# isl-org/Open3D-PointNet2-Semantic3D

Measured on AMD Instinct MI355X. Metric: points/sec through SA+FP stack (B=16,N=8192), higher is better.
Workload: dtype f32

## Files before the change

include/pn2_abi.h:

```cpp
#ifndef PN2_ABI_H_
#define PN2_ABI_H_

#include <stddef.h>
#include <stdint.h>

#ifdef __cplusplus
extern "C" {
#endif

#define PN2_ABI_VERSION 2

#define PN2_OK 0
#define PN2_EINVAL (-1)
#define PN2_ENULL (-2)
#define PN2_ERANGE (-3)
#define PN2_EUNSUP (-4)

#define PN2_ARITH_STRICT 0
#define PN2_ARITH_FMA 1
#define PN2_ARITH_FMA_ALT 2

int pn2_abi_version(void);
const char *pn2_build_info(void);
const char *pn2_strerror(int code);
// ... 157 lines not shown

size_t pn2_interpolate_label_workspace_bytes(int num_sparse_points);
int pn2_interpolate_label_with_color(int num_sparse_points, int num_dense_points,
                                     const float *sparse_points, const int *sparse_labels,
                                     const float *dense_points, int *dense_labels,
                                     uint8_t *dense_colors, int knn, void *workspace,
                                     size_t workspace_bytes, void *stream);


int pn2_linear_dgrad(int rows, int cin, int cout, const float *dy, const float *w, float *dx, void *stream);
int pn2_linear_dgrad_bn_grad_stats(int rows, int cin, int cout, const float *dy, const float *w, float *dx,
                                   const float *y_below, const float *gamma, const float *beta, const float *save_mean,
                                   const float *save_invstd, int relu, void *bn_workspace, size_t workspace_bytes,
                                   void *stream);

int pn2_weighted_ce_forward(int rows, int num_class, const float *logits, const void *labels, int label64,
                            const float *weights, float *lse, double *acc, float *loss, void *stream);
int pn2_weighted_ce_backward(int rows, int num_class, const float *logits, const void *labels, int label64,
                             const float *weights, const float *lse, const double *acc, const float *gout,
                             float *dlogits, void *stream);

int pn2_confusion_update(int rows, int num_class, const float *logits, const void *labels, int label64, int *pred,
                         long long *confusion, long long *invalid, const float *loss, double *loss_acc, void *stream);

int pn2_label_confusion(long long n, int num_class, const void *gt, const void *pd, int label64,
                        long long *confusion, long long *dropped, void *stream);

int pn2_dropout(long long n, const float *x, float keep_prob, const long long *state, float *y,
                unsigned char *mask, void *stream);
int pn2_dropout_grad(long long n, const float *dy, const unsigned char *mask, float keep_prob, float *dx,
                     void *stream);

int pn2_relu_grad(long long n, const float *z, const float *dz, float *dx, void *stream);

int pn2_adam_step(long long n, float *params, const float *grads, float *m, float *v, const float *hyper,
                  void *stream);

int pn2_momentum_step(long long n, float *params, const float *grads, float *accum, const float *hyper, void *stream);

int pn2_sa_group_concat(int b, int n, int m, int nsample, int c, const float *xyz, const float *new_xyz,
                        const float *points, const int *idx, float *out, void *stream);


int pn2_scene_extract_z_box(int n, const double *points, int b, const double *centers, double half_x,
                            double half_y, double scene_z_size, int cap, int *out_idx, int *out_cnt,
                            void *stream);

int pn2_scene_sample(int b, int npts, int cap, const double *points, const int *labels, const double *colors,
                     const int *idx, const int *cnt, const unsigned char *mask, double half_x, double half_y,
                     int *out_sel, float *out_centered, double *out_raw, int *out_labels, float *out_colors,
                     int *status, void *stream);

size_t pn2_voxel_downsample_workspace_bytes(int n);
int pn2_voxel_downsample(int n, const double *points, const double *colors, const int *labels, double voxel_size,
                         double *out_points, double *out_colors, int *out_labels, int *out_count, int *status,
                         void *workspace, size_t workspace_bytes, void *stream);

int pn2_dataset_workspace_size(int b, int max_chunks, unsigned long long *bytes);
int pn2_dataset_sample(int b, int npts, int num_scenes, int max_chunks, int use_color, int augment, const double *points,
                       const float *colors, const unsigned char *labels, const int *scene_offsets, const double *scene_cdf,
                       const double *scene_z_size, const float *label_weights, int num_label_weights, double half_x,
                       double half_y, unsigned long long seed, long long *counter, const int *draw_scene,
                       const int *draw_center, const unsigned char *draw_mask, int mask_cap, const double *draw_rot,
                       void *workspace, size_t workspace_bytes, int *out_info, double *out_finfo, int *out_sel,
                       float *out_data, int *out_labels, float *out_weights, void *stream);

int pn2_scene_ingest_workspace_size(int n, unsigned long long *bytes);
int pn2_scene_ingest(int n, const double *points, const double *colors, const int *labels, double *out_points,
                     float *out_colors, unsigned char *out_labels, int *out_perm, double *out_zrange, long long *out_hist,
                     int *status, void *workspace, size_t workspace_bytes, void *stream);

int pn2_fp_mlp_fused_pre(int b, int n, int m, int c1, const float *dist, const int *idx, const float *points1,
                         const float *z, int nlayers, const int *widths, const float *const *w,
                         const float *const *bias, float *y, void *stream);
int pn2_fp_mlp_fused_pre_ld(int b, int n, int m, int c1, const float *dist, const int *idx, const float *points1,
                            int ld_points1, const float *z, int nlayers, const int *widths, const float *const *w,
                            const float *const *bias, float *y, void *stream);

int pn2_fp_mlp_fused_pre_schedule(int b, int n, int m, int c1, const float *dist, const int *idx, const float *points1,
                                  const float *z, int nlayers, const int *widths, const float *const *w,
                                  const float *const *bias, float *y, int schedule, void *stream);

int pn2_set_sa_row_packing(int on);

int pn2_sa_mlp_fused_pre(int b, int n, int m, int nsample, const float *xyz, const float *new_xyz, const float *zf,
                         const int *idx, int nlayers, const int *widths, const float *const *w,
                         const float *const *bias, int pool, float *out, void *stream);

int pn2_fp_mlp_wide_pre(int b, int n, int m, int c1, const float *dist, const int *idx, const float *points1,
                        const float *z, int nlayers, const int *widths, const float *const *w,
                        const float *const *bias, float *y, void *stream);
int pn2_sa_mlp_wide_pre(int b, int n, int m, int nsample, const float *xyz, const float *new_xyz, const float *zf,
                        const int *idx, int nlayers, const int *widths, const float *const *w,
                        const float *const *bias, int pool, float *y, void *stream);

size_t pn2_ball_query_bin_bytes(int n);
int pn2_ball_query_bin(int b, int n, float radius, const float *xyz1, void *workspace, size_t workspace_bytes, void *stream);
int pn2_ball_query_bin_ld(int b, int n, float radius, const float *xyz1, int ld1, void *workspace, size_t workspace_bytes,
                          void *stream);
int pn2_query_ball_point_binned(int b, int n, int m, float radius, int nsample, const float *xyz1, const float *xyz2,
                                const void *bins, int *idx, int *pts_cnt, int arith_mode, void *stream);

int pn2_group_pool(long long rows, int k, int c, int mode, const float *x, const float *gxyz, float *out, void *stream);
int pn2_group_pool_grad(long long rows, int k, int c, int mode, const float *x, const float *gxyz, const float *dout,
                        float *dx, void *stream);

int pn2_bn_relu_forward_deferred(long long rows, int c, const float *y, const float *gamma, const float *beta,
                                 const float *bias, float eps, float decay, int stats_done, float *running_mean,
                                 float *running_var, void *workspace, size_t workspace_bytes, float *save_mean,
                                 float *save_invstd, float *scale, float *shift, void *stream);
int pn2_linear_bn_stats_xf(int rows, int cin, int cout, const float *x_raw, const float *w, float *y, void *bn_workspace,
                           size_t workspace_bytes, const float *a_scale, const float *a_shift, int a_relu, void *stream);
int pn2_linear_wgrad_accumulate_xf(int rows, int cin, int cout, const float *x_raw, const float *dy, float *dw,
                                   const float *a_scale, const float *a_shift, int a_relu, void *stream);

int pn2_linear_narrow(int rows, int cin, int cout, const float *x, const float *w, const float *bias, float *y, void *stream);

int pn2_bn_grad_constants(long long rows, int c, const float *dz, const float *y, const float *gamma, const float *beta,
                          const float *save_mean, const float *save_invstd, int relu, int pool, const float *zmax,
                          const float *ties, const float *ysel, int stats_done, void *workspace, size_t workspace_bytes,
                          float *coef, float *dgamma, float *dbeta, void *stream);
int pn2_bn_relu_forward_pool(long long rows, int c, const float *y, const float *gamma, const float *beta, const float *bias,
                             float eps, float decay, int relu, int pool, float *running_mean, float *running_var,
                             void *workspace, size_t workspace_bytes, int stats_mode, float *save_mean, float *save_invstd,
                             float *zmax, float *ties, float *ysel, void *stream);
int pn2_linear_dgrad_gx(int rows, int cin, int cout, const float *y, const float *dz, const float *coef, int relu, int pool,
                        const float *zmax, const float *ties, const float *w, float *dx, const float *y_below,
                        const float *gamma_below, const float *beta_below, const float *mean_below, const float *invstd_below,
                        int relu_below, void *ws_below, size_t ws_below_bytes, void *stream);
int pn2_linear_wgrad_gx(int rows, int cin, int cout, const float *x, const float *a_scale, const float *a_shift, int a_relu,
                        const float *y, const float *dz, const float *coef, int relu, int pool, const float *zmax,
                        const float *ties, float *dw, void *stream);

int pn2_linear_bn_stats_fin(int rows, int cin, int cout, const float *x, const float *w, float *y, void *bn_workspace,
                            size_t workspace_bytes, const float *a_scale, const float *a_shift, int a_relu, int finish,
                            const float *gamma, const float *beta, const float *bias, float eps, float decay,
                            float *running_mean, float *running_var, float *save_mean, float *save_invstd, float *scale,
                            float *shift, void *stream);
int pn2_linear_dgrad_fin(int rows, int cin, int cout, const float *dy, const float *y, const float *dz, const float *coef,
                         int relu, int pool, const float *zmax, const float *ties, const float *w, float *dx,
                         const float *y_below, const float *gamma_below, const float *beta_below, const float *mean_below,
                         const float *invstd_below, int relu_below, void *ws_below, size_t ws_below_bytes, int finish_below,
                         float *coef_below, float *dgamma_below, float *dbeta_below, void *stream);
int pn2_bn_relu_forward_mode(long long rows, int c, const float *y, const float *gamma, const float *beta, const float *bias,
                             float eps, float decay, int relu, float *running_mean, float *running_var, void *workspace,
                             size_t workspace_bytes, int stats_mode, float *save_mean, float *save_invstd, float *z,
                             void *stream);
int pn2_bn_relu_backward_mode(long long rows, int c, const float *dz, const float *y, const float *gamma, const float *beta,
                              const float *save_mean, const float *save_invstd, int relu, int pool, const float *zmax,
                              const float *ties, void *workspace, size_t workspace_bytes, int stats_mode, float *dy,
                              float *dgamma, float *dbeta, void *stream);

int pn2_linear_bwd_fused(int rows, int cin, int cout, const float *x, const float *a_scale, const float *a_shift, int a_relu,
                         const float *y, const float *dz, const float *coef, int relu, int pool, const float *zmax,
                         const float *ties, const float *w, float *dx, float *dw, const float *y_below,
                         const float *gamma_below, const float *beta_below, const float *mean_below, const float *invstd_below,
                         int relu_below, void *ws_below, size_t ws_below_bytes, int finish_below, float *coef_below,
                         float *dgamma_below, float *dbeta_below, void *stream);

int pn2_sa_first_layer_bn(int b, int n, int m, int nsample, int c, int cout, const float *xyz, const float *new_xyz,
                          const float *points, const int *idx, const float *w, float *y, float *xg, void *workspace,
                          size_t workspace_bytes, int finish, const float *gamma, const float *beta, const float *bias, float eps,
                          float decay, float *running_mean, float *running_var, float *save_mean, float *save_invstd,
                          float *scale, float *shift, void *stream);

int pn2_sa_hoist_rows(int b, int n, int m, int nsample, int cout, const float *xyz, const float *new_xyz, const int *idx,
// ... 134 lines not shown
```

open3d-pointnet2-semantic3d_amd/csrc/pn2_mlp_wide.hip:

```cpp
#include "pn2_common.h"
#include "pn2_layer_stack.h"

namespace {

typedef float f32x4 __attribute__((ext_vector_type(4)));
typedef float f32x16 __attribute__((ext_vector_type(16)));

constexpr int kWideDepth = 4;

struct WideParams {
    int rows, cin, x_stride, nlayers, pool, relu_last;
    int w[3];
    const float* x;
    int n, m, c;
    const float* xyz;
    const float* new_xyz;
    const float* points;
    const int* idx;
    const float* dist;
    const float* points1;
    int c1, c2;
    const float* W[3];
    const float* bias[3];
    float* y;
    const float* zpre;
    int rowtab_off;
    int sa[2];
    int scratch_off;
    int scratch_alias;
};

enum { kWidePlain = 0, kWideGather = 1, kWideInterp = 2 };
constexpr int kPackChunk = 256;
constexpr int kPackRows = 0, kPackGroups = 32, kPackMeta = 36, kPackCounts = 40, kPackLdsInts = 64;
template <int MODE, bool PACK = false>
__global__ void __launch_bounds__(256, 2)
mlp_wide_kernel(WideParams p) {
    constexpr bool GATHER = MODE == kWideGather;
    static_assert(!PACK || GATHER, "PACK: the pooled gather mode only");
    extern __shared__ __attribute__((aligned(16))) float smem[];
    const int tid = threadIdx.x;
    const int lane = tid & 63, half = lane >> 5, l31 = lane & 31;
    const int wave = __builtin_amdgcn_readfirstlane(tid >> 6);
    const int tile = blockIdx.x;
    const int row0 = tile * 32;
    const int buf_off[2] = {0, 32 * p.sa[0]};
    float* const buf0 = smem;

    struct LayerCfg { int N, wnt, ks_n, nq, ks, cb, g0, g1; const float* wcol; };
    auto make_cfg = [&](int l, int Kt) {
        LayerCfg c;
        c.N = p.w[l];
        c.wnt = c.N >> 7;
        c.ks_n = 4 / c.wnt;
        c.nq = wave % c.wnt;
        c.ks = wave / c.wnt;
        c.cb = c.nq * 128;
        const int ngroups = (Kt + 7) >> 3;
        c.g0 = (ngroups * c.ks) / c.ks_n;
        c.g1 = (ngroups * (c.ks + 1)) / c.ks_n;
        c.wcol = p.W[l] + c.cb + 4 * l31;
        return c;
    };
    f32x4 bq[kWideDepth][4];
    auto fetch_b = [&](const LayerCfg& c, int g, f32x4 (&b_)[4]) {
        const float* __restrict__ wp = c.wcol + (size_t)(8 * g + 4 * half) * c.N;
#pragma unroll
        for (int q = 0; q < 4; ++q) b_[q] = *reinterpret_cast<const f32x4*>(wp + (size_t)q * c.N);
    };
    auto prefetch_b = [&](const LayerCfg& c) {
#pragma unroll
        for (int u = 0; u < kWideDepth; ++u) fetch_b(c, c.g0 + u < c.g1 ? c.g0 + u : c.g1 - 1, bq[u]);
    };
    const LayerCfg first = make_cfg(0, p.cin);
    int* const pk = reinterpret_cast<int*>(smem + p.rowtab_off);
    (void)pk;
    if constexpr (PACK) {
        const int groups = p.rows >> 5;
        const int cbase = (tile / kPackChunk) * kPackChunk, mytile = tile - cbase;
        const int cnt = min(kPackChunk, groups - cbase);
        int cls = 0;
        if (tid < cnt) {
            const int4* __restrict__ ip = reinterpret_cast<const int4*>(p.idx + (size_t)(cbase + tid) * 32);
            int4 v[8];
#pragma unroll
            for (int u = 0; u < 8; ++u) v[u] = ip[u];
            const int head = v[0].x;
            int live = 1;
#pragma unroll
            for (int u = 0; u < 8; ++u) {
                if (v[u].x != head) live = 4 * u + 1;
                if (v[u].y != head) live = 4 * u + 2;
                if (v[u].z != head) live = 4 * u + 3;
                if (v[u].w != head) live = 4 * u + 4;
            }
            cls = live <= 8 ? 8 : (live <= 16 ? 16 : 32);
        }
        const unsigned long long m32 = __ballot(cls == 32), m16 = __ballot(cls == 16), m8 = __ballot(cls == 8);
        if (lane == 0) {
            pk[kPackCounts + 3 * wave + 0] = __popcll(m32);
            pk[kPackCounts + 3 * wave + 1] = __popcll(m16);
            pk[kPackCounts + 3 * wave + 2] = __popcll(m8);
        }
        __syncthreads();
        int n32 = 0, n16 = 0, n8 = 0, b32 = 0, b16 = 0, b8 = 0;
#pragma unroll
        for (int w = 0; w < 4; ++w) {
            const int c32 = pk[kPackCounts + 3 * w], c16 = pk[kPackCounts + 3 * w + 1], c8 = pk[kPackCounts + 3 * w + 2];
            n32 += c32; n16 += c16; n8 += c8;
            if (w < wave) { b32 += c32; b16 += c16; b8 += c8; }
        }
        n32 = __builtin_amdgcn_readfirstlane(n32); n16 = __builtin_amdgcn_readfirstlane(n16); n8 = __builtin_amdgcn_readfirstlane(n8);
        const int promote = ((n16 & 1) && (n8 & 3) == 1) ? 1 : 0;
        const int k16 = n16 + promote, k8 = n8 - promote, t16 = (k16 + 1) >> 1;
        const int ntiles = n32 + t16 + ((k8 + 3) >> 2);
        if (mytile >= ntiles) return;
        prefetch_b(first);
        if (cls != 0) {
            const unsigned long long below = (1ull << lane) - 1ull;
            int t, slot;
            if (cls == 32) { t = b32 + __popcll(m32 & below); slot = 0; }
            else {
                int c = cls, r = cls == 16 ? b16 + __popcll(m16 & below) : b8 + __popcll(m8 & below);
                if (promote && c == 8 && r == n8 - 1) { c = 16; r = n16; }
                if (c == 16) { t = n32 + (r >> 1); slot = r & 1; }
                else { t = n32 + t16 + (r >> 2); slot = r & 3; }
            }
            if (t == mytile) pk[kPackGroups + slot] = cbase + tid;
        }
        if (tid == 0) {
            int sshift, nvalid;
            if (mytile < n32) { sshift = 5; nvalid = 1; }
            else if (mytile < n32 + t16) { sshift = 4; nvalid = min(2, k16 - 2 * (mytile - n32)); }
            else { sshift = 3; nvalid = min(4, k8 - 4 * (mytile - n32 - t16)); }
            pk[kPackMeta] = sshift; pk[kPackMeta + 1] = nvalid;
        }
        __syncthreads();
    } else {
        prefetch_b(first);
    }

    const int K0 = (p.cin + 7) & ~7;
    auto stage4 = [&](int count4, int cv, int sa, auto src_of) {
        for (int base = 0; base < count4; base += 256 * 8) {
            f32x4 v[8];
#pragma unroll
            for (int u = 0; u < 8; ++u) {
                int e = base + u * 256 + tid;
                e = e < count4 ? e : count4 - 1;
                const int r = e / cv, j = e - r * cv;
                v[u] = *reinterpret_cast<const f32x4*>(src_of(r, j));
            }
#pragma unroll
            for (int u = 0; u < 8; ++u) {
                const int e = base + u * 256 + tid;
// ... 75 lines not shown
            for (int u = 0; u < 4; ++u) {
                const int e = base + u * 256 + tid;
                if (e < count4) {
                    const int r = e / cv2, j = e - r * cv2;
                    *reinterpret_cast<f32x4*>(buf0 + r * p.sa[0] + 4 * j) = v[u];
                }
            }
        }
        if (c1 > 0) {
            const float* __restrict__ p1 = p.points1 + (size_t)row0 * c1;
            for (int e = tid; e < 32 * cv1; e += 256) {
                const int r = e / cv1, j = e - r * cv1;
                *reinterpret_cast<f32x4*>(buf0 + r * p.sa[0] + (p.zpre ? 0 : c2) + 4 * j) = *reinterpret_cast<const f32x4*>(p1 + (size_t)r * c1 + 4 * j);
            }
        }
        if (K0 > p.cin) {
            const int padw = K0 - p.cin;
            for (int e = tid; e < 32 * padw; e += 256) buf0[(e / padw) * p.sa[0] + p.cin + e % padw] = 0.f;
        }
    } else {
        const float* __restrict__ x = p.x;
        if ((p.x_stride & 3) == 0 && (p.cin & 3) == 0 && (((uintptr_t)x) & 15) == 0) {
            const int cv = p.cin >> 2;
            stage4(32 * cv, cv, p.sa[0], [&](int r, int j) {
                const int gr = row0 + r < p.rows ? row0 + r : p.rows - 1;
                return x + (size_t)gr * p.x_stride + 4 * j;
            });
            if (row0 + 32 > p.rows) {
                __syncthreads();
                for (int e = tid; e < 32 * p.cin; e += 256) {
                    const int r = e / p.cin;
                    if (row0 + r >= p.rows) buf0[r * p.sa[0] + e - r * p.cin] = 0.f;
                }
            }
        } else {
            const int total = 32 * p.cin;
            for (int base = 0; base < total; base += 256 * 8) {
                float v[8];
#pragma unroll
                for (int u = 0; u < 8; ++u) {
                    int e = base + u * 256 + tid;
                    e = e < total ? e : total - 1;
                    const int r = e / p.cin, k = e - r * p.cin;
                    const int gr = row0 + r < p.rows ? row0 + r : p.rows - 1;
                    v[u] = x[(size_t)gr * p.x_stride + k];
                }
#pragma unroll
                for (int u = 0; u < 8; ++u) {
                    const int e = base + u * 256 + tid;
                    if (e < total) {
                        const int r = e / p.cin, k = e - r * p.cin;
                        buf0[r * p.sa[0] + k] = row0 + r < p.rows ? v[u] : 0.f;
                    }
                }
            }
        }
        if (K0 > p.cin) {
            const int padw = K0 - p.cin;
            for (int e = tid; e < 32 * padw; e += 256) buf0[(e / padw) * p.sa[0] + p.cin + e % padw] = 0.f;
        }
    }
    __syncthreads();

    LayerCfg cur = first;
#pragma unroll 1
    for (int l = 0; l < p.nlayers; ++l) {
        const int N = cur.N, wnt = cur.wnt, ks_n = cur.ks_n, nq = cur.nq, ks = cur.ks, cb = cur.cb, g0 = cur.g0, g1 = cur.g1;
        const int in_off = buf_off[l & 1];
        const int sin = p.sa[l & 1];
        const float* __restrict__ arow = smem + in_off + l31 * sin + 4 * half;

        f32x16 acc[4];
#pragma unroll
        for (int t = 0; t < 4; ++t)
#pragma unroll
            for (int r = 0; r < 16; ++r) acc[t][r] = 0.f;

        auto contract = [&](const f32x4& a_, const f32x4 (&b_)[4]) {
#pragma unroll
            for (int q = 0; q < 4; ++q)
#pragma unroll
                for (int t = 0; t < 4; ++t) acc[t] = __builtin_amdgcn_mfma_f32_32x32x2f32(a_[q], b_[q][t], acc[t], 0, 0, 0);
        };
        if (g0 < g1) {
            const int last = g1 - 1;
            f32x4 aq[kWideDepth];
#pragma unroll
            for (int u = 0; u < kWideDepth; ++u) aq[u] = *reinterpret_cast<const f32x4*>(arow + 8 * (g0 + u < g1 ? g0 + u : last));
            int g = g0;
            for (; g + 2 * kWideDepth <= g1; g += kWideDepth) {
#pragma unroll
                for (int u = 0; u < kWideDepth; ++u) {
                    contract(aq[u], bq[u]);
                    __builtin_amdgcn_sched_barrier(0);
                    const int gn = g + kWideDepth + u;
                    aq[u] = *reinterpret_cast<const f32x4*>(arow + 8 * gn);
                    fetch_b(cur, gn, bq[u]);
                    __builtin_amdgcn_sched_barrier(0);
                }
            }
            const int rem = g1 - g - kWideDepth;
#pragma unroll
            for (int u = 0; u < kWideDepth; ++u) {
                if (g + u < g1) contract(aq[u], bq[u]);
                if (u < rem) {
                    aq[u] = *reinterpret_cast<const f32x4*>(arow + 8 * (g + kWideDepth + u));
                    fetch_b(cur, g + kWideDepth + u, bq[u]);
                }
            }
#pragma unroll
            for (int u = 0; u < kWideDepth - 1; ++u)
                if (u < rem) contract(aq[u], bq[u]);
        }
        const bool lastl = l == p.nlayers - 1;
        LayerCfg nxt = cur;
        if (!lastl) {
            nxt = make_cfg(l + 1, N);
            prefetch_b(nxt);
        }

        if (ks_n > 1) {
            const int sc_off = p.scratch_alias ? in_off : p.scratch_off;
            if (p.scratch_alias) __syncthreads();
            auto park = [&](int block) {
                float* dst = smem + sc_off + block * (64 * 64);
#pragma unroll
                for (int t = 0; t < 4; ++t)
#pragma unroll
                    for (int r = 0; r < 16; ++r) dst[(t * 16 + r) * 64 + lane] = acc[t][r];
            };
            auto add = [&](int block) {
                const float* src = smem + sc_off + block * (64 * 64);
#pragma unroll
                for (int t = 0; t < 4; ++t)
#pragma unroll
                    for (int r = 0; r < 16; ++r) acc[t][r] += src[(t * 16 + r) * 64 + lane];
            };
            if (ks_n == 4) {
                if (ks >= 2) park(ks - 2);
                __syncthreads();
                if (ks < 2) add(ks);
                __syncthreads();
                if (ks == 1) park(0);
                __syncthreads();
                if (ks == 0) add(0);
            } else {
                if (ks == 1) park(nq);
                __syncthreads();
                if (ks == 0) add(nq);
            }
        }
        if (ks == 0 && l == 0 && p.zpre) {
            if constexpr (MODE == kWideInterp) {
                const float* __restrict__ zb = p.zpre + (size_t)(row0 / p.n) * p.m * N + cb + 4 * l31;
                const float* rowtab = smem + p.rowtab_off;
#pragma unroll
                for (int r = 0; r < 16; ++r) {
                    const int row = (r & 3) + 8 * (r >> 2) + 4 * half;
                    const f32x4 wq = *reinterpret_cast<const f32x4*>(rowtab + row * 8);
                    const f32x4 iq = *reinterpret_cast<const f32x4*>(rowtab + row * 8 + 4);
                    const f32x4 z1 = *reinterpret_cast<const f32x4*>(zb + (size_t)__float_as_int(iq[0]) * N);
                    const f32x4 z2 = *reinterpret_cast<const f32x4*>(zb + (size_t)__float_as_int(iq[1]) * N);
                    const f32x4 z3 = *reinterpret_cast<const f32x4*>(zb + (size_t)__float_as_int(iq[2]) * N);
                    const f32x4 z = (z1 * wq[0] + z2 * wq[1]) + z3 * wq[2];
#pragma unroll
                    for (int t = 0; t < 4; ++t) acc[t][r] += z[t];
                }
            } else if constexpr (MODE == kWideGather) {
                const float* __restrict__ zb = p.zpre + (PACK ? (size_t)0 : (size_t)(tile / p.m) * p.n * N) + cb + 4 * l31;
                const int* __restrict__ idx = PACK ? pk + kPackRows : p.idx + (size_t)tile * 32;
#pragma unroll
                for (int r = 0; r < 16; ++r) {
                    const int row = (r & 3) + 8 * (r >> 2) + 4 * half;
                    const f32x4 z = *reinterpret_cast<const f32x4*>(zb + (size_t)idx[row] * N);
#pragma unroll
                    for (int t = 0; t < 4; ++t) acc[t][r] += z[t];
                }
            }
        }
        if (ks == 0) {
            const f32x4 bv = *reinterpret_cast<const f32x4*>(p.bias[l] + cb + 4 * l31);
            const bool relu = !lastl || p.relu_last;
            if (!lastl) {
                float* __restrict__ out = smem + buf_off[(l + 1) & 1];
                const int so = p.sa[(l + 1) & 1];
#pragma unroll
                for (int r = 0; r < 16; ++r) {
                    const int row = (r & 3) + 8 * (r >> 2) + 4 * half;
                    f32x4 v = {acc[0][r] + bv[0], acc[1][r] + bv[1], acc[2][r] + bv[2], acc[3][r] + bv[3]};
                    v = {fmaxf(v[0], 0.f), fmaxf(v[1], 0.f), fmaxf(v[2], 0.f), fmaxf(v[3], 0.f)};
                    *reinterpret_cast<f32x4*>(out + row * so + cb + 4 * l31) = v;
                }
            } else if constexpr (PACK) {
                const int sshift = __builtin_amdgcn_readfirstlane(pk[kPackMeta]);
                const int nvalid = __builtin_amdgcn_readfirstlane(pk[kPackMeta + 1]);
                f32x4 qm[4];
#pragma unroll
                for (int q = 0; q < 4; ++q)
#pragma unroll
                    for (int t = 0; t < 4; ++t) {
                        const float mx = fmaxf(fmaxf(acc[t][4 * q], acc[t][4 * q + 1]), fmaxf(acc[t][4 * q + 2], acc[t][4 * q + 3]));
                        qm[q][t] = fmaxf(mx, __shfl_xor(mx, 32));
                    }
                auto store = [&](int slot, const f32x4& mx) {
                    if (half == 0 && slot < nvalid) {
                        f32x4 v = mx + bv;
                        if (relu) v = {fmaxf(v[0], 0.f), fmaxf(v[1], 0.f), fmaxf(v[2], 0.f), fmaxf(v[3], 0.f)};
                        const int g = pk[kPackGroups + slot];
                        *reinterpret_cast<f32x4*>(p.y + (size_t)g * N + cb + 4 * l31) = v;
                    }
                };
                auto vmax = [](const f32x4& a, const f32x4& b) {
                    return f32x4{fmaxf(a[0], b[0]), fmaxf(a[1], b[1]), fmaxf(a[2], b[2]), fmaxf(a[3], b[3])};
                };
                if (sshift == 3) {
#pragma unroll
                    for (int q = 0; q < 4; ++q) store(q, qm[q]);
                } else if (sshift == 4) {
                    store(0, vmax(qm[0], qm[1]));
                    store(1, vmax(qm[2], qm[3]));
                } else {
                    store(0, vmax(vmax(qm[0], qm[1]), vmax(qm[2], qm[3])));
                }
            } else if (p.pool == 32) {
                f32x4 v;
#pragma unroll
                for (int t = 0; t < 4; ++t) {
                    float mx = acc[t][0];
#pragma unroll
                    for (int r = 1; r < 16; ++r) mx = fmaxf(mx, acc[t][r]);
                    mx = fmaxf(mx, __shfl_xor(mx, 32));
                    mx += bv[t];
                    v[t] = relu ? fmaxf(mx, 0.f) : mx;
                }
                if (half == 0) *reinterpret_cast<f32x4*>(p.y + (size_t)tile * N + cb + 4 * l31) = v;
            } else {
#pragma unroll
                for (int r = 0; r < 16; ++r) {
                    const int row = row0 + (r & 3) + 8 * (r >> 2) + 4 * half;
                    f32x4 v = {acc[0][r] + bv[0], acc[1][r] + bv[1], acc[2][r] + bv[2], acc[3][r] + bv[3]};
                    if (relu) v = {fmaxf(v[0], 0.f), fmaxf(v[1], 0.f), fmaxf(v[2], 0.f), fmaxf(v[3], 0.f)};
                    if (row < p.rows) *reinterpret_cast<f32x4*>(p.y + (size_t)row * N + cb + 4 * l31) = v;
                }
            }
        }
        if (!lastl) __syncthreads();
        cur = nxt;
    }
}

template <int MODE, bool PACK = false>
int launch_mlp_wide_mode(const WideParams& p, size_t lds, hipStream_t st) {
    if (int e = pn2_allow_lds<mlp_wide_kernel<MODE, PACK>>(kPn2CuLdsBytes)) return e;
    mlp_wide_kernel<MODE, PACK><<<(p.rows + 31) / 32, 256, lds, st>>>(p);
    PN2_RETURN_IF_LAUNCH_FAILED();
    return PN2_OK;
}

int launch_mlp_wide(WideParams& p, int mode, hipStream_t st) {
    const int k0 = (p.cin + 7) & ~7;
    int ka = k0, kb = 0;
    if (p.nlayers >= 2) kb = p.w[0];
    if (p.nlayers >= 3 && p.w[1] > ka) ka = p.w[1];
    p.sa[0] = ka + 4;
    p.sa[1] = kb + 4 > 8 ? kb + 4 : 8;
    bool sliced = false, alias_ok = true;
    int kin = k0;
    for (int l = 0; l < p.nlayers; ++l) {
        if (p.w[l] < 512) {
            sliced = true;
            if ((size_t)32 * p.sa[l & 1] < (size_t)2 * 64 * 64) alias_ok = false;
        }
        kin = p.w[l];
    }
    (void)kin;
    p.scratch_off = 32 * (p.sa[0] + p.sa[1]);
    p.scratch_alias = sliced && alias_ok;
    p.rowtab_off = p.scratch_off + (sliced && !alias_ok ? 2 * 64 * 64 : 0);
    const bool pack = mode == kWideGather && p.pool == 32 && pn2_sa_row_packing_enabled() && (((uintptr_t)p.idx) & 15) == 0 &&
                      (long long)(p.rows / 32 / p.m) * p.n <= 0x7fffffffLL;
    const size_t lds = sizeof(float) * ((size_t)p.rowtab_off + (p.zpre && mode == kWideInterp ? 32 * 8 : 0) + (pack ? kPackLdsInts : 0));
    if (lds > kPn2CuLdsBytes) return PN2_EUNSUP;
    if (pack) return launch_mlp_wide_mode<kWideGather, true>(p, lds, st);
    if (mode == kWideGather) return launch_mlp_wide_mode<kWideGather>(p, lds, st);
    if (mode == kWideInterp) return launch_mlp_wide_mode<kWideInterp>(p, lds, st);
    return launch_mlp_wide_mode<kWidePlain>(p, lds, st);
}

constexpr Pn2LayerRule kWideLayers = {3, kPn2WidthsWide, kPn2AlignWeightsAndBias, false};

int fill_wide(WideParams& p, long long rows, int cin, int nlayers, const int* widths, const float* const* w,
              const float* const* bias, int pool, int relu_last, float* y, int between = PN2_OK) {
    if (int rc = pn2_read_layers(p, kWideLayers, nlayers, widths, w, bias)) return rc;
    if (between != PN2_OK) return between;
    if (rows + 64 > 0x7fffffffLL) return PN2_ERANGE;
    p.rows = (int)rows; p.cin = cin; p.nlayers = nlayers; p.pool = pool; p.relu_last = relu_last; p.y = y;
    return PN2_OK;
}

}

extern "C" int pn2_mlp_wide(int rows, int cin, int x_stride, const float* x, int nlayers, const int* widths,
                            const float* const* w, const float* const* bias, int relu_last, int pool, float* y, void* stream) {
    if (rows <= 0 || cin <= 0 || x_stride < cin) return PN2_EINVAL;
    if (!x || !y) return PN2_ENULL;
    const int own = (pool != 0 && pool != 32) ? PN2_EUNSUP
                    : (pool == 32 && rows % 32 != 0) ? PN2_EINVAL
                    : (((uintptr_t)y) & 15) ? PN2_EUNSUP : PN2_OK;
    WideParams p = {};
    if (int rc = fill_wide(p, rows, cin, nlayers, widths, w, bias, pool, relu_last, y, own)) return rc;
    p.x_stride = x_stride; p.x = x;
    return launch_mlp_wide(p, kWidePlain, static_cast<hipStream_t>(stream));
}

extern "C" int pn2_sa_mlp_wide(int b, int n, int m, int nsample, int c, const float* xyz, const float* new_xyz,
                               const float* points, const int* idx, int nlayers, const int* widths, const float* const* w,
                               const float* const* bias, int pool, float* y, void* stream) {
    if (b <= 0 || n <= 0 || m <= 0 || c <= 0) return PN2_EINVAL;
    if (!xyz || !new_xyz || !points || !idx || !y) return PN2_ENULL;
    if (nsample != 32 || c % 4 != 0 || (((uintptr_t)points | (uintptr_t)y) & 15)) return PN2_EUNSUP;
    WideParams p = {};
    if (int rc = fill_wide(p, (long long)b * m * 32, 3 + c, nlayers, widths, w, bias, pool ? 32 : 0, 1, y)) return rc;
    p.n = n; p.m = m; p.c = c; p.xyz = xyz; p.new_xyz = new_xyz; p.points = points; p.idx = idx;
    return launch_mlp_wide(p, kWideGather, static_cast<hipStream_t>(stream));
}

extern "C" int pn2_fp_mlp_wide(int b, int n, int m, int c1, int c2, const float* dist, const int* idx, const float* points1,
                               const float* points2, int nlayers, const int* widths, const float* const* w,
                               const float* const* bias, float* y, void* stream) {
    if (b <= 0 || n <= 0 || m < 3 || c2 <= 0 || c1 < 0) return PN2_EINVAL;
    if (!dist || !idx || !points2 || !y || (c1 > 0 && !points1)) return PN2_ENULL;
    if (n % 32 != 0 || c2 % 4 != 0 || c1 % 4 != 0 || (((uintptr_t)points2 | (uintptr_t)points1 | (uintptr_t)y) & 15)) return PN2_EUNSUP;
    WideParams p = {};
    if (int rc = fill_wide(p, (long long)b * n, c2 + c1, nlayers, widths, w, bias, 0, 1, y)) return rc;
    p.n = n; p.m = m; p.c1 = c1; p.c2 = c2; p.dist = dist; p.idx = idx; p.points = points2; p.points1 = points1;
    return launch_mlp_wide(p, kWideInterp, static_cast<hipStream_t>(stream));
}

extern "C" int pn2_fp_mlp_wide_pre(int b, int n, int m, int c1, const float* dist, const int* idx, const float* points1,
                                   const float* z, int nlayers, const int* widths, const float* const* w,
                                   const float* const* bias, float* y, void* stream) {
    if (b <= 0 || n <= 0 || m < 3 || c1 <= 0) return PN2_EINVAL;
    if (!dist || !idx || !z || !y || !points1) return PN2_ENULL;
    if (n % 32 != 0 || c1 % 4 != 0 || (((uintptr_t)z | (uintptr_t)points1 | (uintptr_t)y) & 15)) return PN2_EUNSUP;
    WideParams p = {};
    if (int rc = fill_wide(p, (long long)b * n, c1, nlayers, widths, w, bias, 0, 1, y)) return rc;
    p.n = n; p.m = m; p.c1 = c1; p.c2 = 0; p.dist = dist; p.idx = idx; p.points1 = points1; p.zpre = z;
    return launch_mlp_wide(p, kWideInterp, static_cast<hipStream_t>(stream));
}

extern "C" int pn2_sa_mlp_wide_pre(int b, int n, int m, int nsample, const float* xyz, const float* new_xyz, const float* zf,
                                   const int* idx, int nlayers, const int* widths, const float* const* w,
                                   const float* const* bias, int pool, float* y, void* stream) {
    if (b <= 0 || n <= 0 || m <= 0) return PN2_EINVAL;
    if (!xyz || !new_xyz || !zf || !idx || !y) return PN2_ENULL;
    if (nsample != 32 || (((uintptr_t)zf | (uintptr_t)y) & 15)) return PN2_EUNSUP;
    WideParams p = {};
    if (int rc = fill_wide(p, (long long)b * m * 32, 3, nlayers, widths, w, bias, pool ? 32 : 0, 1, y)) return rc;
    p.n = n; p.m = m; p.c = 4; p.xyz = xyz; p.new_xyz = new_xyz; p.points = zf; p.idx = idx; p.zpre = zf;
    return launch_mlp_wide(p, kWideGather, static_cast<hipStream_t>(stream));
}
```

open3d-pointnet2-semantic3d_amd/util/pointnet_util.py:

```python

import torch

from . import tf_util
from .._lib import float_array, int_array, launch, lib, ptr, ptr_table, require_cuda, rows_in_place, u64_array
from ..tf_ops import tf_grouping
from ..tf_ops.tf_grouping import query_ball_point_multi, group_point, knn_point, query_ball_point
from ..tf_ops.tf_interpolate import three_interpolate, three_nn
from ..tf_ops.tf_sampling import (farthest_point_sample, farthest_point_sample_and_gather, farthest_point_sample_with_ties,
                                  gather_point, tag_fps_output)

USE_FUSED_SA = True
USE_HOISTED_SA = True
USE_SA_ROW_PACKING = True
_sa_row_packing_told = True
USE_HOISTED_FP = True
USE_FUSED_TRAIN_FRONT = True
USE_MLP_CHAIN = True
USE_MLP_WIDE = True
WIDE_MIN_ROWS = 4096
USE_FUSED_FP = True
_WIDE_WIDTHS = (128, 256, 512)


def sample_and_group(npoint, radius, nsample, xyz, points, knn=False, use_xyz=True, geometry=None):
    plan = None
    if geometry is not None:
        new_xyz, idx = geometry[0], geometry[1]
        plan = geometry[2] if len(geometry) > 2 else None
    else:
        fps_idx, fps_tie, _ = farthest_point_sample_with_ties(npoint, xyz)
        new_xyz = tag_fps_output(gather_point(xyz, fps_idx), fps_tie)
        if knn:
            _, idx = knn_point(nsample, xyz, new_xyz)
        else:
            idx, pts_cnt = query_ball_point(radius, nsample, xyz, new_xyz)
    if USE_FUSED_TRAIN_FRONT and points is not None and use_xyz and points.dtype == torch.float32:
        if points.requires_grad and torch.is_grad_enabled():
            new_points = _SAGroupConcat.apply(xyz.contiguous(), new_xyz.contiguous(), points.contiguous(), idx, plan)
        else:
            new_points = _sa_group_concat(xyz.detach().contiguous(), new_xyz.detach().contiguous(), points.detach(), idx)
        return new_xyz, new_points, idx, new_points[..., :3]
    grouped_xyz = group_point(xyz, idx)
    grouped_xyz = grouped_xyz - new_xyz.unsqueeze(2)
    if points is not None:
        grouped_points = group_point(points, idx)
        if use_xyz:
            new_points = torch.cat([grouped_xyz, grouped_points], dim=-1)
        else:
            new_points = grouped_points
    else:
        new_points = grouped_xyz
    return new_xyz, new_points, idx, grouped_xyz


def sample_and_group_all(xyz, points, use_xyz=True):
    b, n, _ = xyz.shape
    new_xyz = torch.zeros((b, 1, 3), dtype=torch.float32, device=xyz.device)
    idx = torch.arange(n, dtype=torch.int32, device=xyz.device).reshape(1, 1, n).repeat(b, 1, 1)
    grouped_xyz = xyz.reshape(b, 1, n, 3)
    if points is not None:
        new_points = torch.cat([xyz, points], dim=2) if use_xyz else points
        new_points = new_points.unsqueeze(1)
    else:
        new_points = grouped_xyz
    return new_xyz, new_points, idx, grouped_xyz


def _sa_fused_inference(xyz, new_xyz, points, idx, mlp, bn, conv_scope_fmt, pool=True, xyz_last=False):
    b, n, _ = xyz.shape
    m, nsample = idx.shape[1], idx.shape[2]
    c = 0 if points is None else points.shape[2]
    bf16 = points is not None and points.dtype == torch.bfloat16
    if bf16:
        if not pool or nsample not in (32, 64) or c % 16 != 0:
            return None
    elif nsample != 32 and (not pool or nsample not in (16, 64, 128, 256)):
        return None
    if len(mlp) > 3 or any(w % 32 != 0 or w > 128 for w in mlp):
        return None
    ws, bs = [], []
    cin = 3 + c
    for i, cout in enumerate(mlp):
        with tf_util.variable_scope(conv_scope_fmt % i):
            w2, b2 = tf_util.folded_dense(cin, cout, bn, (1, 1, cin, cout),
                                          rotate_rows=3 if (xyz_last and i == 0 and c > 0) else 0)
        ws.append(w2)
        bs.append(b2)
        cin = cout
    _sync_sa_row_packing(xyz)
    oshape = (b, m, mlp[-1]) if pool else (b, m, nsample, mlp[-1])
    if (USE_HOISTED_SA and not bf16 and nsample == 32 and c >= 32 and c % 4 == 0
            and ((pool and tuple(mlp) in ((64, 64, 128), (128, 128, 128))) or (not pool and tuple(mlp) == (128, 128)))):
        w1x, w1f = tf_util.split_first_layer(ws[0], 3, c, "sa_pre")
        xyz, points = xyz.contiguous(), points.contiguous()
        zf = tf_util.hoist_gemm(points.reshape(b * n, c), w1f)
        out = tf_util._launch_stack("pn2_sa_mlp_fused_pre", xyz, (b, n, m, nsample, xyz, new_xyz, zf, idx), ws, bs,
                                    (int(bool(pool)),), oshape, w0=w1x)
        if out is not None:
            return out
    xyz_v, ldx = rows_in_place(xyz)
    pts, ldp = (None, 0) if points is None else rows_in_place(points)
    if pool and not bf16 and (ldx != 3 or (points is not None and ldp != c)):
# ... 139 lines not shown

def coarse_geometry_fits(n0, npoints, want_nn=True):
    if not USE_COARSE_GEOMETRY or not (0 < n0 <= COARSE_MAX_N) or not (0 < len(npoints) <= COARSE_MAX_LEVELS):
        return False
    n = n0
    for m in npoints:
        if not (0 < m <= n) or (want_nn and not (3 <= m <= COARSE_MAX_NN_M)):
            return False
        n = m
    return True


def coarse_geometry(xyz0, npoints, radii, nsamples, want_nn=True, fps_arith_mode=None, bq_arith_mode=None):
    from .. import config
    from ..tf_ops.tf_sampling import fps_tie_record
    require_cuda(xyz0)
    if xyz0.dim() != 3 or xyz0.shape[2] != 3 or xyz0.dtype != torch.float32:
        raise ValueError("coarse_geometry expects (batch_size,num_points,3) float32 xyz0")
    nlev = len(npoints)
    if not (len(radii) == len(nsamples) == nlev):
        raise ValueError("coarse_geometry expects one radius and one nsample per level")
    tie_in = fps_tie_record(xyz0, fps_arith_mode)
    xyz0 = xyz0.detach().contiguous()
    b, n0, _ = xyz0.shape
    dev = xyz0.device
    out, n = [], n0
    for m, ns in zip(npoints, nsamples):
        lv = {"new_xyz": torch.empty((b, m, 3), dtype=torch.float32, device=dev),
              "fps_idx": torch.empty((b, m), dtype=torch.int32, device=dev),
              "idx": torch.empty((b, m, ns), dtype=torch.int32, device=dev),
              "cnt": torch.empty((b, m), dtype=torch.int32, device=dev),
              "nn": (torch.empty((b, n, 3), dtype=torch.float32, device=dev),
                     torch.empty((b, n, 3), dtype=torch.int32, device=dev)) if want_nn else None}
        out.append(lv)
        n = m
    tie_out = torch.empty((b,), dtype=torch.int32, device=dev)
    launch("pn2_coarse_geometry", dev, b, n0, nlev, int_array(npoints), float_array(radii), int_array(nsamples), ptr(xyz0), ptr(tie_in),
           ptr_table([lv["fps_idx"] for lv in out]), ptr_table([lv["new_xyz"] for lv in out]), ptr_table([lv["idx"] for lv in out]),
           ptr_table([lv["cnt"] for lv in out]), ptr_table([lv["nn"][0] if want_nn else None for lv in out]),
           ptr_table([lv["nn"][1] if want_nn else None for lv in out]), ptr(tie_out), config.fps_mode(fps_arith_mode),
           config.bq_mode(bq_arith_mode))
    tag_fps_output(out[-1]["new_xyz"], tie_out, fps_arith_mode)
    return out


def _first_taken(routes, *args):
    for route in routes:
        got = route(*args)
        if got is not None:
            return got
    raise AssertionError("unreachable: the last route takes every configuration")


class _SaCall:

    def __init__(self, xyz, new_xyz, points, idx, mlp, bn, bn_decay):
        self.xyz, self.new_xyz, self.points, self.idx = xyz, new_xyz, points, idx
        self.mlp, self.bn, self.bn_decay, self.nsample = mlp, bn, bn_decay, idx.shape[2]
        self.was_bf16 = False


def _sa_route_mlp_max_fused(a):
    if not USE_FUSED_SA:
        return None
    return _sa_fused_inference(a.xyz, a.new_xyz, a.points, a.idx, a.mlp, a.bn, "conv%d")


def _sa_step_dense_float32(a):
    a.xyz = a.xyz.contiguous()
    a.points = None if a.points is None else a.points.contiguous()
    if a.points is not None and a.points.dtype == torch.bfloat16:
        a.points, a.was_bf16 = a.points.float(), True
    return None


def _sa_route_mlp_max_fused_float32(a):
    return _sa_route_mlp_max_fused(a) if a.was_bf16 else None


def _sa_route_mlp_rows_fused(a):
    mlp = a.mlp
    if not (USE_FUSED_SA and len(mlp) == 3 and mlp[0] == mlp[1] == 128 and mlp[2] % 32 == 0):
        return None
    h = _sa_fused_inference(a.xyz, a.new_xyz, a.points, a.idx, mlp[:2], a.bn, "conv%d", pool=False)
    if h is None:
        return None
    h = tf_util.conv2d(h, mlp[2], [1, 1], padding="VALID", stride=[1, 1], bn=a.bn, is_training=False,
                       scope="conv2", bn_decay=a.bn_decay, pool=a.nsample)
    return h.squeeze(2)


def _sa_wide_layers(a):
    mlp, points = a.mlp, a.points
    if not (USE_MLP_WIDE and USE_FUSED_SA and a.nsample == 32 and points is not None
            and points.dtype == torch.float32 and points.shape[2] % 4 == 0 and 1 <= len(mlp) <= 3
            and all(w in _WIDE_WIDTHS for w in mlp) and a.idx.shape[0] * a.idx.shape[1] * 32 >= WIDE_MIN_ROWS):
        return None
    folded, cprev = [], 3 + points.shape[2]
    for i, cout in enumerate(mlp):
        with tf_util.variable_scope("conv%d" % i):
            if i == 0:
                folded.append(tf_util.folded_dense(cprev, cout, a.bn, (1, 1, cprev, cout), pad_to=32,
                                                   pad_in=-(-cprev // 8) * 8, rotate_rows=cprev - 3))
            else:
                folded.append(tf_util.folded_dense(cprev, cout, a.bn, (1, 1, cprev, cout), pad_to=32))
        cprev = cout
    _sync_sa_row_packing(a.xyz)
    return [f[0] for f in folded], [f[1] for f in folded]


def _sa_route_mlp_wide_pre(a):
    layers = _sa_wide_layers(a) if USE_HOISTED_SA else None
    return None if layers is None else tf_util.hip_sa_mlp_wide_pre(a.xyz, a.new_xyz, a.points, a.idx, *layers)


def _sa_route_mlp_wide(a):
    layers = _sa_wide_layers(a)
    return None if layers is None else tf_util.hip_sa_mlp_wide(a.xyz, a.new_xyz, a.points, a.idx, *layers)


def _sa_route_group_concat(a):
    h = _sa_group_concat(a.xyz, a.new_xyz, a.points, a.idx)
    pool_ok = a.nsample == 16 or a.nsample % 32 == 0
    for i, cout in enumerate(a.mlp):
        last = i == len(a.mlp) - 1
        h = tf_util.conv2d(h, cout, [1, 1], padding="VALID", stride=[1, 1], bn=a.bn, is_training=False,
                           scope="conv%d" % i, bn_decay=a.bn_decay, pool=a.nsample if (last and pool_ok) else 0)
    if not pool_ok:
        h = h.amax(dim=2, keepdim=True)
    return h.squeeze(2)


SA_ROUTES = (_sa_route_mlp_max_fused, _sa_step_dense_float32, _sa_route_mlp_max_fused_float32, _sa_route_mlp_rows_fused,
             _sa_route_mlp_wide_pre, _sa_route_mlp_wide, _sa_route_group_concat)


def sa_features_inference(xyz, new_xyz, points, idx, mlp, bn=True, bn_decay=None):
    return _first_taken(SA_ROUTES, _SaCall(xyz, new_xyz, points, idx, mlp, bn, bn_decay))


_POOL_MODES = {"max": 0, "avg": 1, "weighted_avg": 2, "max_and_avg": 3}


class _GroupPool(torch.autograd.Function):
    @staticmethod
    def forward(ctx, x, gxyz, mode):
        b, m, k, c = x.shape
        x = x.contiguous()
        gxyz = gxyz.contiguous() if gxyz is not None else None
        out = torch.empty((b, m, 1, 2 * c if mode == 3 else c), dtype=torch.float32, device=x.device)
        launch("pn2_group_pool", x, b * m, k, c, mode, ptr(x), ptr(gxyz), ptr(out))
        ctx.save_for_backward(x, gxyz if gxyz is not None else x.new_empty(0))
        ctx.mode = mode
        return out

    @staticmethod
    def backward(ctx, dout):
        x, gxyz = ctx.saved_tensors
        b, m, k, c = x.shape
        dx = torch.empty_like(x)
        launch("pn2_group_pool_grad", x, b * m, k, c, ctx.mode, ptr(x), ptr(gxyz if gxyz.numel() else None), ptr(dout.contiguous()),
               ptr(dx))
        return dx, None, None


def group_pool(new_points, grouped_xyz, pooling):
    mode = _POOL_MODES[pooling]
    require_cuda(new_points)
    if new_points.dtype != torch.float32:
        raise TypeError("pooling expects float32 features")
    tf_util.assert_not_deferred(new_points, "a pooling")
    return _GroupPool.apply(new_points, grouped_xyz if mode == 2 else None, mode)


def _sa_first_layer_fusable(is_training, points, mlp, nsample, group_all, knn, use_xyz, bn, pooling):
    return (bool(is_training) and not group_all and not knn and use_xyz and bn and pooling == "max" and points is not None
            and points.dtype == torch.float32 and len(mlp) > 0 and mlp[0] % 4 == 0 and nsample <= 1024)


# ... 342 lines not shown
```

Measured before the change: 384.2 million.

## Keep K-split partial sums in registers for 128-wide gather layers

For the gather (SA) mode, 128-wide layers now give each of the four waves a 32-column slice and a full-K contraction. Each wave's weights are loaded as scalar rows and its four K sub-slices are accumulated in separate MFMA accumulators, which are then summed in registers. This removes the LDS park/reduce step and its barriers that the K-split path needed. The epilogue (zpre add, bias, ReLU, pooling, packed stores) is rewritten for the single-column-per-lane layout. It also adds a runtime toggle and a Python routing hook with an SA3 threshold, set very high so that routing stays off by default.

Result: no change. 382.5 million (-0.5%).

```diff
diff --git a/include/pn2_abi.h b/include/pn2_abi.h
--- a/include/pn2_abi.h
+++ b/include/pn2_abi.h
@@ -263,6 +263,8 @@
                                   const float *const *bias, float *y, int schedule, void *stream);
 
 int pn2_set_sa_row_packing(int on);
+
+int pn2_set_wide_slices(int in_registers);
 
 int pn2_sa_mlp_fused_pre(int b, int n, int m, int nsample, const float *xyz, const float *new_xyz, const float *zf,
                          const int *idx, int nlayers, const int *widths, const float *const *w,
diff --git a/open3d-pointnet2-semantic3d_amd/csrc/pn2_mlp_wide.hip b/open3d-pointnet2-semantic3d_amd/csrc/pn2_mlp_wide.hip
--- a/open3d-pointnet2-semantic3d_amd/csrc/pn2_mlp_wide.hip
+++ b/open3d-pointnet2-semantic3d_amd/csrc/pn2_mlp_wide.hip
@@ -1,5 +1,6 @@
 #include "pn2_common.h"
 #include "pn2_layer_stack.h"
+#include <atomic>
 
 namespace {
 
@@ -28,6 +29,7 @@
     int sa[2];
     int scratch_off;
     int scratch_alias;
+    int reg_slices;
 };
 
 enum { kWidePlain = 0, kWideGather = 1, kWideInterp = 2 };
@@ -37,6 +39,7 @@
 __global__ void __launch_bounds__(256, 2)
 mlp_wide_kernel(WideParams p) {
     constexpr bool GATHER = MODE == kWideGather;
+    constexpr bool kRegs = GATHER;
     static_assert(!PACK || GATHER, "PACK: the pooled gather mode only");
     extern __shared__ __attribute__((aligned(16))) float smem[];
     const int tid = threadIdx.x;
@@ -47,7 +50,7 @@
     const int buf_off[2] = {0, 32 * p.sa[0]};
     float* const buf0 = smem;
 
-    struct LayerCfg { int N, wnt, ks_n, nq, ks, cb, g0, g1; const float* wcol; };
+    struct LayerCfg { int N, wnt, ks_n, nq, ks, cb, g0, g1, ng, regs; const float* wcol; };
     auto make_cfg = [&](int l, int Kt) {
         LayerCfg c;
         c.N = p.w[l];
@@ -57,9 +60,12 @@
         c.ks = wave / c.wnt;
         c.cb = c.nq * 128;
         const int ngroups = (Kt + 7) >> 3;
+        c.ng = ngroups;
         c.g0 = (ngroups * c.ks) / c.ks_n;
         c.g1 = (ngroups * (c.ks + 1)) / c.ks_n;
         c.wcol = p.W[l] + c.cb + 4 * l31;
+        c.regs = kRegs && p.reg_slices != 0 && c.ks_n == 4;
+        if (c.regs) c.wcol = p.W[l] + 4 * half * 128 + 32 * wave + l31;
         return c;
     };
     f32x4 bq[kWideDepth][4];
@@ -68,9 +74,33 @@
 #pragma unroll
         for (int q = 0; q < 4; ++q) b_[q] = *reinterpret_cast<const f32x4*>(wp + (size_t)q * c.N);
     };
+    auto slice_g0 = [](int ng, int s) { return (ng * s) >> 2; };
+    auto slice_extra = [](int ng, int s) { return (((ng * (s + 1)) >> 2) - ((ng * s) >> 2)) - (ng >> 2); };
+    auto fetch_rows = [&](const LayerCfg& c, int g, f32x4& b_) {
+        const float* __restrict__ wp = c.wcol + (size_t)(8 * g) * 128;
+#pragma unroll
+        for (int q = 0; q < 4; ++q) b_[q] = wp[q * 128];
+    };
+    auto fetch_short = [&](const LayerCfg& c, f32x4 (&b_)[4]) {
+#pragma unroll
+        for (int s = 0; s < 4; ++s) fetch_rows(c, slice_g0(c.ng, s), b_[s]);
+    };
+    auto fetch_full = [&](const LayerCfg& c, int f, f32x4 (&b_)[4]) {
+#pragma unroll
+        for (int s = 0; s < 4; ++s) fetch_rows(c, slice_g0(c.ng, s) + slice_extra(c.ng, s) + f, b_[s]);
+    };
     auto prefetch_b = [&](const LayerCfg& c) {
-#pragma unroll
-        for (int u = 0; u < kWideDepth; ++u) fetch_b(c, c.g0 + u < c.g1 ? c.g0 + u : c.g1 - 1, bq[u]);
+        if (kRegs && c.regs) {
+            const int nfull = c.ng >> 2;
+            if (c.ng & 3) fetch_short(c, bq[0]);
+            else fetch_full(c, 0, bq[0]);
+#pragma unroll
+            for (int u = 1; u < kWideDepth; ++u)
+                if (u < nfull) fetch_full(c, u, bq[u]);
+            return;
+        }
+#pragma unroll
+        for (int u = 0; u < kWideDepth; ++u) fetch_b(c, c.g0 + u < c.g1 ? c.g0 + u : max(c.g1 - 1, 0), bq[u]);
     };
     const LayerCfg first = make_cfg(0, p.cin);
     int* const pk = reinterpret_cast<int*>(smem + p.rowtab_off);
@@ -312,7 +342,59 @@
 #pragma unroll
                 for (int t = 0; t < 4; ++t) acc[t] = __builtin_amdgcn_mfma_f32_32x32x2f32(a_[q], b_[q][t], acc[t], 0, 0, 0);
         };
-        if (g0 < g1) {
+        if (kRegs && cur.regs) {
+            const int ng = cur.ng, nfull = ng >> 2;
+            f32x4 ar[4];
+            auto read_pair = [&](int h, int f) {
+#pragma unroll
+                for (int s = 2 * h; s < 2 * h + 2; ++s)
+                    ar[s] = *reinterpret_cast<const f32x4*>(arow + 8 * min(slice_g0(ng, s) + slice_extra(ng, s) + f, ng - 1));
+            };
+            auto contract_pair = [&](int h, const f32x4 (&b_)[4]) {
+#pragma unroll
+                for (int q = 0; q < 4; ++q)
+#pragma unroll
+                    for (int s = 2 * h; s < 2 * h + 2; ++s) acc[s] = __builtin_amdgcn_mfma_f32_32x32x2f32(ar[s][q], b_[s][q], acc[s], 0, 0, 0);
+            };
+            if (ng & 3) {
+#pragma unroll
+                for (int s = 0; s < 4; ++s) ar[s] = *reinterpret_cast<const f32x4*>(arow + 8 * slice_g0(ng, s));
+#pragma unroll
+                for (int s = 0; s < 4; ++s)
+                    if (slice_extra(ng, s)) {
+#pragma unroll
+                        for (int q = 0; q < 4; ++q) acc[s] = __builtin_amdgcn_mfma_f32_32x32x2f32(ar[s][q], bq[0][s][q], acc[s], 0, 0, 0);
+                    }
+                if (nfull > 0) fetch_full(cur, 0, bq[0]);
+            }
+            if (nfull > 0) {
+                read_pair(0, 0);
+                read_pair(1, 0);
+                int f = 0;
+                for (; f + kWideDepth <= nfull; f += kWideDepth) {
+#pragma unroll
+                    for (int u = 0; u < kWideDepth; ++u) {
+                        contract_pair(0, bq[u]);
+                        __builtin_amdgcn_sched_barrier(0);
+                        read_pair(0, f + u + 1);
+                        __builtin_amdgcn_sched_barrier(0);
+                        contract_pair(1, bq[u]);
+                        __builtin_amdgcn_sched_barrier(0);
+                        read_pair(1, f + u + 1);
+                        if (f + u + kWideDepth < nfull) fetch_full(cur, f + u + kWideDepth, bq[u]);
+                        __builtin_amdgcn_sched_barrier(0);
+                    }
+                }
+#pragma unroll
+                for (int u = 0; u < kWideDepth - 1; ++u)
+                    if (f + u < nfull) {
+                        contract_pair(0, bq[u]);
+                        read_pair(0, f + u + 1);
+                        contract_pair(1, bq[u]);
+                        read_pair(1, f + u + 1);
+                    }
+            }
+        } else if (g0 < g1) {
             const int last = g1 - 1;
             f32x4 aq[kWideDepth];
 #pragma unroll
@@ -349,7 +431,11 @@
             prefetch_b(nxt);
         }
 
-        if (ks_n > 1) {
+        if (kRegs && cur.regs) {
+            acc[0] += acc[2];
+            acc[1] += acc[3];
+            acc[0] += acc[1];
+        } else if (ks_n > 1) {
             const int sc_off = p.scratch_alias ? in_off : p.scratch_off;
             if (p.scratch_alias) __syncthreads();
             auto park = [&](int block) {
@@ -380,13 +466,78 @@
                 if (ks == 0) add(nq);
             }
         }
-        if (ks == 0 && l == 0 && p.zpre) {
+        int hrow = half;
+        if constexpr (kRegs) asm volatile("" : "+v"(hrow));
+        if constexpr (kRegs) {
+            if (cur.regs) {
+                const int col = 32 * wave + l31;
+                if (l == 0 && p.zpre) {
+                    const float* __restrict__ zb = p.zpre + (PACK ? (size_t)0 : (size_t)(tile / p.m) * p.n * N) + col;
+                    const int* __restrict__ idx = PACK ? pk + kPackRows : p.idx + (size_t)tile * 32;
+                    float z[16];
+#pragma unroll
+                    for (int r = 0; r < 16; ++r) z[r] = zb[(size_t)idx[(r & 3) + 8 * (r >> 2) + 4 * hrow] * N];
+                    __builtin_amdgcn_sched_barrier(0);
+#pragma unroll
+                    for (int r = 0; r < 16; ++r) acc[0][r] += z[r];
+                }
+                const float bv = p.bias[l][col];
+                const bool relu = !lastl || p.relu_last;
+                if (!lastl) {
+                    float* __restrict__ out = smem + buf_off[(l + 1) & 1] + col;
+                    const int so = p.sa[(l + 1) & 1];
+#pragma unroll
+                    for (int r = 0; r < 16; ++r) out[((r & 3) + 8 * (r >> 2) + 4 * hrow) * so] = fmaxf(acc[0][r] + bv, 0.f);
+                } else if constexpr (PACK) {
+                    const int sshift = __builtin_amdgcn_readfirstlane(pk[kPackMeta]);
+                    const int nvalid = __builtin_amdgcn_readfirstlane(pk[kPackMeta + 1]);
+                    float qm[4];
+#pragma unroll
+                    for (int q = 0; q < 4; ++q) {
+                        const float mx = fmaxf(fmaxf(acc[0][4 * q], acc[0][4 * q + 1]), fmaxf(acc[0][4 * q + 2], acc[0][4 * q + 3]));
+                        qm[q] = fmaxf(mx, __shfl_xor(mx, 32));
+                    }
+                    auto store = [&](int slot, float mx) {
+                        if (half == 0 && slot < nvalid) {
+                            float v = mx + bv;
+                            if (relu) v = fmaxf(v, 0.f);
+                            p.y[(size_t)pk[kPackGroups + slot] * N + col] = v;
+                        }
+                    };
+                    if (sshift == 3) {
+#pragma unroll
+                        for (int q = 0; q < 4; ++q) store(q, qm[q]);
+                    } else if (sshift == 4) {
+                        store(0, fmaxf(qm[0], qm[1]));
+                        store(1, fmaxf(qm[2], qm[3]));
+                    } else {
+                        store(0, fmaxf(fmaxf(qm[0], qm[1]), fmaxf(qm[2], qm[3])));
+                    }
+                } else if (p.pool == 32) {
+                    float mx = acc[0][0];
+#pragma unroll
+                    for (int r = 1; r < 16; ++r) mx = fmaxf(mx, acc[0][r]);
+                    mx = fmaxf(mx, __shfl_xor(mx, 32));
+                    mx += bv;
+                    if (half == 0) p.y[(size_t)tile * N + col] = relu ? fmaxf(mx, 0.f) : mx;
+                } else {
+#pragma unroll
+                    for (int r = 0; r < 16; ++r) {
+                        const int row = row0 + (r & 3) + 8 * (r >> 2) + 4 * hrow;
+                        float v = acc[0][r] + bv;
+                        if (relu) v = fmaxf(v, 0.f);
+                        if (row < p.rows) p.y[(size_t)row * N + col] = v;
+                    }
+                }
+            }
+        }
+        if (!(kRegs && cur.regs) && ks == 0 && l == 0 && p.zpre) {
             if constexpr (MODE == kWideInterp) {
                 const float* __restrict__ zb = p.zpre + (size_t)(row0 / p.n) * p.m * N + cb + 4 * l31;
                 const float* rowtab = smem + p.rowtab_off;
 #pragma unroll
                 for (int r = 0; r < 16; ++r) {
-                    const int row = (r & 3) + 8 * (r >> 2) + 4 * half;
+                    const int row = (r & 3) + 8 * (r >> 2) + 4 * hrow;
                     const f32x4 wq = *reinterpret_cast<const f32x4*>(rowtab + row * 8);
                     const f32x4 iq = *reinterpret_cast<const f32x4*>(rowtab + row * 8 + 4);
                     const f32x4 z1 = *reinterpret_cast<const f32x4*>(zb + (size_t)__float_as_int(iq[0]) * N);
@@ -401,14 +552,14 @@
                 const int* __restrict__ idx = PACK ? pk + kPackRows : p.idx + (size_t)tile * 32;
 #pragma unroll
                 for (int r = 0; r < 16; ++r) {
-                    const int row = (r & 3) + 8 * (r >> 2) + 4 * half;
+                    const int row = (r & 3) + 8 * (r >> 2) + 4 * hrow;
                     const f32x4 z = *reinterpret_cast<const f32x4*>(zb + (size_t)idx[row] * N);
 #pragma unroll
                     for (int t = 0; t < 4; ++t) acc[t][r] += z[t];
                 }
             }
         }
-        if (ks == 0) {
+        if (!(kRegs && cur.regs) && ks == 0) {
             const f32x4 bv = *reinterpret_cast<const f32x4*>(p.bias[l] + cb + 4 * l31);
             const bool relu = !lastl || p.relu_last;
             if (!lastl) {
@@ -416,7 +567,7 @@
                 const int so = p.sa[(l + 1) & 1];
 #pragma unroll
                 for (int r = 0; r < 16; ++r) {
-                    const int row = (r & 3) + 8 * (r >> 2) + 4 * half;
+                    const int row = (r & 3) + 8 * (r >> 2) + 4 * hrow;
                     f32x4 v = {acc[0][r] + bv[0], acc[1][r] + bv[1], acc[2][r] + bv[2], acc[3][r] + bv[3]};
                     v = {fmaxf(v[0], 0.f), fmaxf(v[1], 0.f), fmaxf(v[2], 0.f), fmaxf(v[3], 0.f)};
                     *reinterpret_cast<f32x4*>(out + row * so + cb + 4 * l31) = v;
@@ -467,7 +618,7 @@
             } else {
 #pragma unroll
                 for (int r = 0; r < 16; ++r) {
-                    const int row = row0 + (r & 3) + 8 * (r >> 2) + 4 * half;
+                    const int row = row0 + (r & 3) + 8 * (r >> 2) + 4 * hrow;
                     f32x4 v = {acc[0][r] + bv[0], acc[1][r] + bv[1], acc[2][r] + bv[2], acc[3][r] + bv[3]};
                     if (relu) v = {fmaxf(v[0], 0.f), fmaxf(v[1], 0.f), fmaxf(v[2], 0.f), fmaxf(v[3], 0.f)};
                     if (row < p.rows) *reinterpret_cast<f32x4*>(p.y + (size_t)row * N + cb + 4 * l31) = v;
@@ -478,6 +629,8 @@
         cur = nxt;
     }
 }
+
+std::atomic<int> g_wide_slices{1};
 
 template <int MODE, bool PACK = false>
 int launch_mlp_wide_mode(const WideParams& p, size_t lds, hipStream_t st) {
@@ -494,10 +647,11 @@
     if (p.nlayers >= 3 && p.w[1] > ka) ka = p.w[1];
     p.sa[0] = ka + 4;
     p.sa[1] = kb + 4 > 8 ? kb + 4 : 8;
+    p.reg_slices = mode == kWideGather && g_wide_slices.load(std::memory_order_relaxed) != 0;
     bool sliced = false, alias_ok = true;
     int kin = k0;
     for (int l = 0; l < p.nlayers; ++l) {
-        if (p.w[l] < 512) {
+        if (p.w[l] < 512 && !(p.reg_slices && p.w[l] == 128)) {
             sliced = true;
             if ((size_t)32 * p.sa[l & 1] < (size_t)2 * 64 * 64) alias_ok = false;
         }
@@ -530,6 +684,11 @@
 
 }
 
+extern "C" int pn2_set_wide_slices(int in_registers) {
+    g_wide_slices.store(in_registers != 0, std::memory_order_relaxed);
+    return PN2_OK;
+}
+
 extern "C" int pn2_mlp_wide(int rows, int cin, int x_stride, const float* x, int nlayers, const int* widths,
                             const float* const* w, const float* const* bias, int relu_last, int pool, float* y, void* stream) {
     if (rows <= 0 || cin <= 0 || x_stride < cin) return PN2_EINVAL;
diff --git a/open3d-pointnet2-semantic3d_amd/util/pointnet_util.py b/open3d-pointnet2-semantic3d_amd/util/pointnet_util.py
--- a/open3d-pointnet2-semantic3d_amd/util/pointnet_util.py
+++ b/open3d-pointnet2-semantic3d_amd/util/pointnet_util.py
@@ -18,6 +18,7 @@
 USE_MLP_CHAIN = True
 USE_MLP_WIDE = True
 WIDE_MIN_ROWS = 4096
+SA3_WIDE_MIN_ROWS = 1 << 30
 USE_FUSED_FP = True
 _WIDE_WIDTHS = (128, 256, 512)
 
@@ -323,6 +324,9 @@
     mlp = a.mlp
     if not (USE_FUSED_SA and len(mlp) == 3 and mlp[0] == mlp[1] == 128 and mlp[2] % 32 == 0):
         return None
+    if (tuple(mlp) == (128, 128, 256) and a.idx.shape[0] * a.idx.shape[1] * 32 >= SA3_WIDE_MIN_ROWS and _sa_wide_takes(a)
+            and a.points.shape[2] == 128):
+        return None
     h = _sa_fused_inference(a.xyz, a.new_xyz, a.points, a.idx, mlp[:2], a.bn, "conv%d", pool=False)
     if h is None:
         return None
@@ -331,11 +335,16 @@
     return h.squeeze(2)
 
 
+def _sa_wide_takes(a):
+    mlp, points = a.mlp, a.points
+    return bool(USE_MLP_WIDE and USE_FUSED_SA and a.nsample == 32 and points is not None
+                and points.dtype == torch.float32 and points.shape[2] % 4 == 0 and 1 <= len(mlp) <= 3
+                and all(w in _WIDE_WIDTHS for w in mlp) and a.idx.shape[0] * a.idx.shape[1] * 32 >= WIDE_MIN_ROWS)
+
+
 def _sa_wide_layers(a):
     mlp, points = a.mlp, a.points
-    if not (USE_MLP_WIDE and USE_FUSED_SA and a.nsample == 32 and points is not None
-            and points.dtype == torch.float32 and points.shape[2] % 4 == 0 and 1 <= len(mlp) <= 3
-            and all(w in _WIDE_WIDTHS for w in mlp) and a.idx.shape[0] * a.idx.shape[1] * 32 >= WIDE_MIN_ROWS):
+    if not _sa_wide_takes(a):
         return None
     folded, cprev = [], 3 + points.shape[2]
     for i, cout in enumerate(mlp):
```
